# orjfickel/Small-Project-UV-Robot-Ray-Tracer

Measured on AMD Instinct MI355X. Metric: Mray/s (extend+shade) on C046_1.glb 1920x1080x8-bounce, higher is better.
Workload: dtype f32; 1 GPU; testroomopt.glb (stand-in for the absent rooms/C046_1.glb), 2073600 photons/launch x 8 waves, lamp 0 of lange_route.xml, SEED_0=0; step = reset + generate + extend of all waves (batched), accumulate + shade replayed per wave + sync; triangles=44866, mode=batched, launch_pipelining=True, flavour=0, seed_mode=0, wide_bvh=False, parallelism=1 GPU, self_comm=False, high_priority_stream=False, full=False

## Files before the change

small-project-uv-robot-ray-tracer_amd/csrc/uvrt_kernels.hip:

```cpp
#include "uvrt_device.h"

namespace uvrt {


__device__ __forceinline__ uint32_t coherence_key(uint32_t qphi, uint32_t qy, uint32_t qo,
                                                  int bphi, int by, int bo)
{
    uint32_t key = 0;
    while (bphi > 0 || by > 0 || bo > 0) {
        if (bphi > 0) { --bphi; key = (key << 1) | ((qphi >> bphi) & 1u); }
        if (by > 0) { --by; key = (key << 1) | ((qy >> by) & 1u); }
        if (bo > 0) { --bo; key = (key << 1) | ((qo >> bo) & 1u); }
    }
    return key;
}

__global__ __launch_bounds__(256) void k_generate(GenParams p)
{
    helper_priority(p.prio);
    if (blockIdx.x >= p.ray_blocks) {
        const int j = (int)(blockIdx.x - p.ray_blocks) * 256 + threadIdx.x;
        if (j < p.prep_npairs) prepare_record6(p.prep_pairs, p.prep_recs, p.lx, p.lz, p.prep_npairs, j, p.prep_perm);
        return;
    }
    const int64_t i = (int64_t)blockIdx.x * 256 + threadIdx.x;
    if (i >= p.n) return;
    const int64_t gid = p.first_gid + i;
    float r0;
    double x, y;
    const float4 ray = generate_ray(p.lx, p.ly, p.lz, p.light_length, gid, p.seed_prev, p.seed_next, p.seed_mode, r0, x, y);
    const float diry = ray.y;
    p.rays[i] = ray;

    if (p.keyrank) {
        const float fx = (float)x, fy = (float)y;
        const float ax = fabsf(fx), ay = fabsf(fy);
        float t = ay / (ax + ay + 1e-30f);
        float ang = fx >= 0.0f ? (fy >= 0.0f ? t : 4.0f - t) : (fy >= 0.0f ? 2.0f - t : 2.0f + t);
        const uint32_t nphi = 1u << p.bits_phi, ny = 1u << p.bits_y, no = 1u << p.bits_o;
        uint32_t qphi = min((uint32_t)(ang * (0.25f * (float)nphi)), nphi - 1);
        uint32_t qy = min((uint32_t)((diry + 1.0f) * (0.5f * (float)ny)), ny - 1);
        uint32_t qo = min((uint32_t)(r0 * (float)no), no - 1);
        const uint32_t key = coherence_key(qphi, qy, qo, p.bits_phi, p.bits_y, p.bits_o);
        const uint32_t rank = atomicAdd(&p.hist[key], 1u);
        p.keyrank[i] = make_uint2(key, rank);
    }
}

__global__ __launch_bounds__(256) void k_generate_batch(GenBatchParams p)
{
    helper_priority(p.prio);
    const int64_t i = (int64_t)blockIdx.x * 256 + threadIdx.x;
    if (i >= p.n) return;
    const int k = blockIdx.y;
    float r0;
    double x, y;
    p.rays[(int64_t)k * p.n_pad + i] = generate_ray(p.lx[k], p.ly[k], p.lz[k], p.light_length, p.first_gid + i,
                                                    p.seed_prev[k], p.seed_next[k], p.seed_mode, r0, x, y);
}

__global__ __launch_bounds__(64) void k_dedupe_mark(GenDedupeParams p)
{
    helper_priority(p.prio);
    constexpr int32_t W = DEDUPE_MARK_KEYS;
    __shared__ uint32_t s_table[W];
    const int lane = threadIdx.x, K = p.g.count;
    const uint32_t nb = (uint32_t)((p.gn + DD_SLOTS - 1) / DD_SLOTS);
    const int32_t lo = (int32_t)(p.g.first_gid > 1 ? p.g.first_gid : 1), hi = (int32_t)(p.g.first_gid + p.g.n);
    const int32_t c0 = (int32_t)p.g0, c1 = (int32_t)(p.g0 + p.gn);
    if ((int32_t)blockIdx.x >= p.gap_strip0[p.gaps]) {
        static_assert(DEDUPE_PERIODIC_WORDS % 64 == 0 && DEDUPE_PERIODIC_WORDS <= W, "the words fit the key table's LDS in whole rounds");
#pragma unroll
        for (int i = 0; i < DEDUPE_PERIODIC_WORDS; i += 64) s_table[i + lane] = p.per.words[i + lane];
        __syncthreads();
        const uint32_t t = (blockIdx.x - (uint32_t)p.gap_strip0[p.gaps]) * 64u + (uint32_t)lane;
        if (t < (uint32_t)K * nb) {
            const uint32_t k = t / nb, b = t - k * nb;
            const int32_t x0 = c0 + (int32_t)(b * (uint32_t)DD_SLOTS), x1 = min(x0 + DD_SLOTS, c1);
            const uint32_t owners = dedupe_periodic_owners(p.g, p.per, s_table, (int)k, max(x0, 1), x1);
            if (owners != 0u) atomicAdd(&p.block_counts[t], owners);
        }
        return;
    }
    int gap = 0;
    while (gap + 1 < p.gaps && (int32_t)blockIdx.x >= p.gap_strip0[gap + 1]) ++gap;
    const int64_t gap_lo = p.gap_key[gap];
    const uint32_t gap_keys = p.gap_keys[gap];
    const int64_t gap_tiles = (int64_t)((gap_keys + (uint32_t)W - 1u) / (uint32_t)W);
    const int64_t tile0 = (int64_t)((int32_t)blockIdx.x - p.gap_strip0[gap]) * p.strip_tiles;
    const int64_t tile1 = tile0 + p.strip_tiles < gap_tiles ? tile0 + p.strip_tiles : gap_tiles;
    int32_t run_lo = hi, run_hi = hi, key0 = 0;
    uint32_t seed1 = 0u;
    if (lane < K) {
        run_lo = dedupe_strip_first(p.g, lane, gap_lo + tile0 * W);
        seed1 = dedupe_seed1(p.g, lane);
        key0 = p.g.key0[lane];
    }
    uint32_t cnt_block = 0u, cnt = 0u;
    const auto add_owners = [&](int j, uint32_t block, uint32_t owners) { atomicAdd(&p.block_counts[(size_t)j * nb + block], owners); };
    const auto count_owners = [&](int j, uint32_t block, uint32_t owners) {
        if (lane == j && owners != 0u) {
            if (block != cnt_block) {
                if (cnt != 0u) add_owners(j, cnt_block, cnt);
                cnt_block = block;
                cnt = 0u;
            }
            cnt += owners;
        }
    };
    for (int64_t tile = tile0; tile < tile1; ++tile) {
        const int64_t t0 = gap_lo + tile * W;
        const int32_t w = (int32_t)min((uint32_t)W, gap_keys - (uint32_t)(tile * W));
        static_assert(W % 64 == 0, "the wave zeroes the table in whole rounds");
#pragma unroll
        for (int i = 0; i < W; i += 64) s_table[i + lane] = 0u;
        __syncthreads();
        for (int j = 0; j < K; ++j) {
            int32_t base = __builtin_amdgcn_readlane(run_lo, j);
            const uint32_t seed = (uint32_t)__builtin_amdgcn_readlane((int)seed1, j);
            for (;;) {
                const int32_t g = base + lane;
                bool in = false;
                if (g < hi) {
                    const int32_t key = dedupe_key1_of(p.g, seed, g);
                    in = dedupe_in_tile(key, t0, w);
                    if (in) dedupe_tile_insert_run(s_table, dedupe_tile_slot(key, t0), j, dedupe_run_twice(p.g, seed, g, key, lo, hi));
                }
                const int32_t n_in = (int32_t)__popcll(__builtin_amdgcn_ballot_w64(in));
                base += n_in;
                if (n_in < 64) break;
            }
            if (lane == j) run_hi = base;
        }
        const bool holds0 = lane < K && dedupe_tile_holds_key0(p.g, key0, t0, w);
        if (holds0) dedupe_tile_insert(s_table, dedupe_tile_slot(key0, t0), lane);
        __syncthreads();
        for (int j = 0; j < K; ++j) {
            const int32_t a = max(__builtin_amdgcn_readlane(run_lo, j), c0), b = min(__builtin_amdgcn_readlane(run_hi, j), c1);
            const uint32_t seed = (uint32_t)__builtin_amdgcn_readlane((int)seed1, j);
            for (int32_t base = a; base < b; base += 64) {
                const int32_t g = base + lane;
                const uint32_t fb = (uint32_t)(base - c0) / (uint32_t)DD_SLOTS;
                uint32_t mask = 0u, blk = fb;
                if (g < b) {
                    const uint32_t slot = dedupe_tile_slot(dedupe_key1_of(p.g, seed, g), t0);
                    mask = dedupe_tile_resolve(slot < (uint32_t)w ? s_table[slot] : DEDUPE_MANY, j);
                    p.tmp[(int64_t)j * p.gn + (g - c0)] = mask;
                    blk = (uint32_t)(g - c0) / (uint32_t)DD_SLOTS;
                }
                const int32_t last = min(base + 63, b - 1);
                if ((uint32_t)(last - c0) / (uint32_t)DD_SLOTS == fb) {
                    count_owners(j, fb, (uint32_t)__popcll(__builtin_amdgcn_ballot_w64(mask != 0u)));
                } else {
                    const uint32_t n0 = (uint32_t)__popcll(__builtin_amdgcn_ballot_w64(mask != 0u && blk == fb));
                    const uint32_t n1 = (uint32_t)__popcll(__builtin_amdgcn_ballot_w64(mask != 0u && blk != fb));
                    count_owners(j, fb, n0);
                    count_owners(j, fb + 1u, n1);
                }
            }
        }
        if (c0 == 0 && holds0) {
            const uint32_t mask = dedupe_tile_resolve(s_table[dedupe_tile_slot(key0, t0)], lane);
            p.tmp[(int64_t)lane * p.gn] = mask;
            if (mask != 0u) add_owners(lane, 0u, 1u);
        }
        run_lo = run_hi;
        __syncthreads();
    }
    if (lane < K && cnt != 0u) add_owners(lane, cnt_block, cnt);
}

__global__ __launch_bounds__(256) void k_dedupe_scan(uint32_t* block_counts, uint32_t* total, uint32_t* deposits, uint32_t nblocks, int prio)
{
    helper_priority(prio);
    __shared__ uint32_t s_part[256];
    const uint32_t tid = threadIdx.x;
    if (tid == 0u) *deposits = 0u;
    const uint32_t per = (nblocks + 255u) / 256u;
    const uint32_t lo = min(tid * per, nblocks), hi = min(lo + per, nblocks);
    uint32_t sum = 0;
    for (uint32_t b = lo; b < hi; ++b) sum += block_counts[b];
    s_part[tid] = sum;
    __syncthreads();
    for (uint32_t off = 1; off < 256u; off <<= 1) {
        const uint32_t v = tid >= off ? s_part[tid - off] : 0u;
        __syncthreads();
        s_part[tid] += v;
        __syncthreads();
    }
    uint32_t run = s_part[tid] - sum;
    for (uint32_t b = lo; b < hi; ++b) {
        const uint32_t c = block_counts[b];
        block_counts[b] = run;
        run += c;
    }
    if (tid == 255u) *total = s_part[255];
}

__global__ __launch_bounds__(256) void k_dedupe_write(GenDedupeParams p)
{
    helper_priority(p.prio);
    __shared__ uint32_t s_cnt[DD_ROUNDS][4];
    __shared__ uint32_t s_slot_mask[DEDUPE_CLASS_SLOTS], s_slot_word[DEDUPE_CLASS_SLOTS], s_dep;
    if (threadIdx.x < (unsigned)DEDUPE_CLASS_SLOTS) {
        s_slot_mask[threadIdx.x] = p.cls.slot_mask[threadIdx.x];
        s_slot_word[threadIdx.x] = p.cls.slot_word[threadIdx.x];
    }
    if (threadIdx.x == 0) s_dep = 0u;
    const bool classes = p.cls.count > 0;
    uint32_t dep = 0u;
    const int k = blockIdx.y;
    const uint32_t wv = threadIdx.x >> 6;
    static_assert(256 % DEDUPE_PERIOD_MAX == 0, "a thread's rounds share their residue");
    uint32_t near = 0u, worded = 0u;
    bool inside = false;
    const uint32_t seed1 = dedupe_seed1(p.g, k);
    const int32_t gid0 = (int32_t)(p.g0 + (int64_t)blockIdx.x * DD_SLOTS) + (int32_t)threadIdx.x;
    if (p.per.count > 0) {
        const int32_t x0 = max((int32_t)(p.g0 + (int64_t)blockIdx.x * DD_SLOTS), 1);
        const int32_t x1 = (int32_t)min(p.g0 + ((int64_t)blockIdx.x + 1) * DD_SLOTS, p.g0 + p.gn);
        const int32_t ka = __builtin_amdgcn_readfirstlane(dedupe_key1_of(p.g, seed1, x0));
        const int32_t kb = __builtin_amdgcn_readfirstlane(dedupe_key1_of(p.g, seed1, x1 - 1));
#pragma unroll
        for (int s = 0; s < DEDUPE_PERIODIC_STRATA; ++s) {
            const int32_t A = p.per.key_lo[s], B = A + (int32_t)p.per.keys[s];
            if (s < p.per.count && kb >= A && ka < B) {
                near |= 1u << s;
                inside = ka >= A && kb < B;
            }
        }
    }
    uint32_t mask[DD_ROUNDS], rank[DD_ROUNDS];
#pragma unroll
    for (int r = 0; r < DD_ROUNDS; ++r) mask[r] = 0u;
    for (uint32_t left = near; left != 0u; left &= left - 1u) {
        const int s = __builtin_ctz(left);
        const int32_t A = p.per.key_lo[s], P = p.per.period[s];
        const uint32_t len = p.per.keys[s];
        const uint32_t* w = &p.per.words[p.per.word_off[s] + k * P];
        const int32_t res = gid0 & (P - 1);
        uint32_t word = 0u;
#pragma unroll
        for (int q = 0; q < DEDUPE_PERIOD_MAX; ++q) {
            const uint32_t wq = w[q];
            if (res == q) word = wq;
        }
#pragma unroll
        for (int r = 0; r < DD_ROUNDS; ++r) {
            const int64_t i = (int64_t)blockIdx.x * DD_SLOTS + r * 256 + threadIdx.x;
            const int32_t g = gid0 + r * 256;
            if (i < p.gn && g >= 1 && (inside || (uint32_t)dedupe_key1_of(p.g, seed1, g) - (uint32_t)A < len)) {
                mask[r] = word;
                worded |= 1u << r;
            }
        }
    }
    uint32_t pos = p.block_counts[(size_t)k * gridDim.x + blockIdx.x];
#pragma unroll
    for (int r = 0; r < DD_ROUNDS; ++r) {
        const int64_t i = (int64_t)blockIdx.x * DD_SLOTS + r * 256 + threadIdx.x;
        if (!((worded >> r) & 1u) && i < p.gn) mask[r] = p.tmp[(int64_t)k * p.gn + i];
        const unsigned long long owners = __builtin_amdgcn_ballot_w64(mask[r] != 0u);
        rank[r] = __builtin_amdgcn_mbcnt_hi((uint32_t)(owners >> 32), __builtin_amdgcn_mbcnt_lo((uint32_t)owners, 0u));
        if ((threadIdx.x & 63u) == 0u) s_cnt[r][wv] = (uint32_t)__popcll(owners);
    }
    __syncthreads();
    if (threadIdx.x == 0) p.block_counts[(size_t)k * gridDim.x + blockIdx.x] = 0u;
#pragma unroll
    for (int r = 0; r < DD_ROUNDS; ++r) {
        for (uint32_t w = 0; w < 4u; ++w) {
            if (w == wv && mask[r] != 0u) {
                const int64_t i = (int64_t)blockIdx.x * DD_SLOTS + r * 256 + threadIdx.x;
                float r0;
                double x, y;
                p.rays[pos + rank[r]] = generate_ray(p.g.lx, p.g.ly, p.g.lz, p.light_length, p.g0 + i, p.g.seed_prev[k],
                                                     p.g.seed_next[k], p.g.seed_mode, r0, x, y);
                const uint32_t word = ((worded >> r) & 1u) ? mask[r] : dedupe_deposit_word(classes, s_slot_mask, s_slot_word, mask[r]);
                p.masks[pos + rank[r]] = word;
                dep += (uint32_t)dedupe_word_deposits(classes, word);
            }
            pos += s_cnt[r][w];
        }
    }
    if (dep != 0u) atomicAdd(&s_dep, dep);
    __syncthreads();
    if (threadIdx.x == 0 && s_dep != 0u) atomicAdd(p.deposits, s_dep);
}

__global__ __launch_bounds__(1024) void k_scan_bins(uint32_t* hist, uint32_t* bin_start,
                                                    int32_t nbins)
{
    __shared__ uint32_t s_part[1024];
    const int tid = threadIdx.x;
    const int per = (nbins + 1023) / 1024;
    const int lo = tid * per, hi = min(lo + per, nbins);
    uint32_t sum = 0;
    for (int b = lo; b < hi; ++b) sum += hist[b];
    s_part[tid] = sum;
    __syncthreads();
    for (int off = 1; off < 1024; off <<= 1) {
        uint32_t v = tid >= off ? s_part[tid - off] : 0u;
        __syncthreads();
        s_part[tid] += v;
        __syncthreads();
    }
    uint32_t run = s_part[tid] - sum;
    for (int b = lo; b < hi; ++b) {
        const uint32_t c = hist[b];
        bin_start[b] = run;
        hist[b] = 0;
        run += c;
    }
}

__global__ __launch_bounds__(256) void k_scatter(const float4* __restrict__ rays,
                                                 const uint2* __restrict__ keyrank,
                                                 const uint32_t* __restrict__ bin_start,
                                                 float4* __restrict__ sorted,
                                                 uint32_t* __restrict__ order, int64_t n)
{
    const int64_t i = (int64_t)blockIdx.x * 256 + threadIdx.x;
    if (i >= n) return;
    const uint2 kr = keyrank[i];
    const uint32_t pos = bin_start[kr.x] + kr.y;
    const float4 r = rays[i];
    sorted[pos] = r;
    order[pos] = (uint32_t)i;
}


__global__ __launch_bounds__(256) void k_accumulate(double* __restrict__ photon_map,
                                                    double* __restrict__ max_map,
                                                    int32_t* __restrict__ counts, int32_t replicas,
                                                    int64_t stride, float time_step, int32_t T, int prio)
{
    helper_priority(prio);
    const int g = blockIdx.x * 256 + threadIdx.x;
    const int i = g >> 2, part = g & 3;
    int32_t total = 0;
    if (i < T) {
        for (int r = part; r < replicas; r += 4) {
            total += counts[r * stride + i];
            counts[r * stride + i] = 0;
        }
    }
    total += __builtin_amdgcn_mov_dpp(total, 0xb1, 0xf, 0xf, true);
    total += __builtin_amdgcn_mov_dpp(total, 0x4e, 0xf, 0xf, true);
    if (i >= T || part != 0) return;
    const double c = (double)total;
    photon_map[i] = photon_map[i] + c * (double)time_step;
    const double m = max_map[i];
    max_map[i] = m < c ? c : m;
}

__global__ __launch_bounds__(256) void k_fold_counts(int32_t* __restrict__ counts, int32_t replicas,
                                                     int64_t stride, int32_t T)
{
    const int i = blockIdx.x * 256 + threadIdx.x;
    if (i >= T) return;
    int32_t total = counts[i];
    for (int r = 1; r < replicas; ++r) {
        total += counts[r * stride + i];
        counts[r * stride + i] = 0;
    }
    counts[i] = total;
}

__device__ __forceinline__ void heatmap(float intensity, float& r, float& g, float& b)
{
    const float minDosageColor = 0.5f;
    const float upperHalfColor = 0.75f;
    const float lowerHalfColor = 0.25f;
    if (intensity > minDosageColor) {
        if (intensity > upperHalfColor) {
            r = 1.0f; g = (1.0f - intensity) / (1.0f - upperHalfColor); b = 0.0f;
        } else {
            r = (intensity - minDosageColor) / (upperHalfColor - minDosageColor);
            g = 1.0f; b = 0.0f;
        }
    } else {
        if (intensity > lowerHalfColor) {
            r = 0.0f; g = 1.0f;
            b = (minDosageColor - intensity) / (minDosageColor - lowerHalfColor);
        } else {
            r = 0.0f; g = intensity / lowerHalfColor; b = 1.0f;
        }
    }
}

__global__ __launch_bounds__(256) void k_fold_planes(int32_t* __restrict__ planes, int32_t* __restrict__ folded,
                                                     int32_t replicas, int32_t T, int prio)
{
    helper_priority(prio);
    const int g = blockIdx.x * 256 + threadIdx.x;
    const int i = g >> 2, part = g & 3;
    int32_t* pl = planes + (int64_t)blockIdx.y * replicas * T;
    int32_t total = 0;
    if (i < T) {
        for (int r = part; r < replicas; r += 4) {
            total += pl[(int64_t)r * T + i];
            pl[(int64_t)r * T + i] = 0;
        }
    }
    total += __builtin_amdgcn_mov_dpp(total, 0xb1, 0xf, 0xf, true);
    total += __builtin_amdgcn_mov_dpp(total, 0x4e, 0xf, 0xf, true);
    if (i < T && part == 0) folded[(int64_t)blockIdx.y * T + i] = total;
}

__device__ __forceinline__ int32_t take_class_plane(int32_t* pl, int32_t replicas, int64_t replica_stride, int i, int part, bool in)
{
    int32_t total = 0;
    if (in) {
        for (int r = part; r < replicas; r += 4) {
            total += pl[(int64_t)r * replica_stride + i];
            pl[(int64_t)r * replica_stride + i] = 0;
        }
    }
    total += __builtin_amdgcn_mov_dpp(total, 0xb1, 0xf, 0xf, true);
    total += __builtin_amdgcn_mov_dpp(total, 0x4e, 0xf, 0xf, true);
    return total;
}

__global__ __launch_bounds__(256) void k_fold_classes(FoldClassParams p)
{
    helper_priority(p.prio);
    const int g = blockIdx.x * 256 + threadIdx.x;
    const int i = g >> 2, part = g & 3;
    const bool in = i < p.T;
    for (int c = 0; c < p.ncls; ++c) {
        const int32_t total = take_class_plane(p.planes + (int64_t)(p.nplanes + c) * p.plane_stride, p.cls_replicas, p.T, i, part, in);
        if (!in || part != 0 || total == 0) continue;
        for (uint64_t m = p.launches[c]; m != 0ull; m &= m - 1ull) p.folded[(int64_t)__builtin_ctzll(m) * p.T + i] += total;
    }
}

__global__ __launch_bounds__(256) void k_replay_batch(ReplayParams p)
{
    helper_priority(p.prio);
    const int g = blockIdx.x * 256 + threadIdx.x;
    const int i = g >> 2, part = g & 3;
    const bool in = i < p.bound;
    double pm = 0, mm = 0;
    if (in && part == 0) { pm = p.photon_map[i]; mm = p.max_map[i]; }
    extern __shared__ int32_t s_cls[];
    const int ncls = p.is_folded ? 0 : p.ncls;
    for (int c = 0; c < ncls; ++c) {
        const int32_t total = take_class_plane(p.planes + (int64_t)(p.nplanes + c) * p.plane_stride, p.cls_replicas, p.T, i, part, in);
        if (part == 0) s_cls[c * 64 + (threadIdx.x >> 2)] = total;
    }
    for (int k = 0; k < p.count; ++k) {
        const ReplayOp op = p.ops[k];
        int32_t total = 0;
        if (p.is_folded) {
            if (in && part == 0) {
                int32_t* f = p.folded + (int64_t)op.plane * p.T + i;
                total = *f;
                *f = 0;
            }
        } else {
            if (in) {
                int32_t* pl = p.planes + (int64_t)op.plane * p.plane_stride;
                for (int r = part; r < p.replicas; r += 4) {
                    total += pl[(int64_t)r * p.T + i];
                    pl[(int64_t)r * p.T + i] = 0;
                }
            }
            total += __builtin_amdgcn_mov_dpp(total, 0xb1, 0xf, 0xf, true);
            total += __builtin_amdgcn_mov_dpp(total, 0x4e, 0xf, 0xf, true);
        }
        if (!in || part != 0) continue;
        if (ncls > 0)
            for (uint64_t m = p.class_of[k]; m != 0ull; m &= m - 1ull) total += s_cls[__builtin_ctzll(m) * 64 + (threadIdx.x >> 2)];
        const double c = (double)total;
        pm = pm + c * (double)op.duration;
        mm = mm < c ? c : mm;
        if (op.shade) {
            const double num = (double)op.scaled_power * (op.which_map ? mm : pm);
            const float den = p.area[i] * (float)op.photons_per_light;
            const float dose = (float)(num / (double)den);
            p.dosage[i] = dose;
            const float maxValue = op.min_value * 2;
            const float norm = dose / maxValue;
            float r, gg, b;
            if (op.threshold_view && norm < 0.5f) { r = 0.0f; gg = 0.0f; b = norm * 2.0f; }
            else heatmap(norm, r, gg, b);
            float* col = p.color + (int64_t)i * 9;
            col[0] = r; col[1] = gg; col[2] = b;
            col[3] = r; col[4] = gg; col[5] = b;
            col[6] = r; col[7] = gg; col[8] = b;
        }
    }
    if (in && part == 0) { p.photon_map[i] = pm; p.max_map[i] = mm; }
}

__global__ __launch_bounds__(256) void k_add_counts(int32_t* __restrict__ dst, const int32_t* __restrict__ src, int64_t n)
{
    const int64_t i = (int64_t)blockIdx.x * 256 + threadIdx.x;
    if (i < n) dst[i] += src[i];
}

__global__ __launch_bounds__(256) void k_reset(double* __restrict__ photon_map,
                                               double* __restrict__ max_map,
                                               int32_t* __restrict__ counts, int32_t replicas,
                                               int64_t stride, float* __restrict__ color,
                                               int32_t reset_color, int32_t T, int prio)
{
    helper_priority(prio);
    const int i = blockIdx.x * 256 + threadIdx.x;
    if (i >= T) return;
    photon_map[i] = 0;
    max_map[i] = 0;
    for (int r = 0; r < replicas; ++r) counts[r * stride + i] = 0;
    if (!reset_color) return;
    for (int k = 0; k < 9; ++k) color[(int64_t)i * 9 + k] = 0.0f;
}

__global__ __launch_bounds__(256) void k_prepare_scene(const float4* __restrict__ tris64,
                                                       const uint32_t* __restrict__ tri_idx,
                                                       LeafTri* __restrict__ ltris,
                                                       float* __restrict__ area, int32_t T)
{
    const int i = blockIdx.x * 256 + threadIdx.x;
    if (i >= T) return;
    {
        const uint32_t id = tri_idx[i];
        const float4 v0 = tris64[(int64_t)id * 4 + 0], v1 = tris64[(int64_t)id * 4 + 1],
                     v2 = tris64[(int64_t)id * 4 + 2];
        LeafTri t;
        t.v0_id = make_float4(v0.x, v0.y, v0.z, __uint_as_float(id));
        t.e1 = make_float4(v1.x - v0.x, v1.y - v0.y, v1.z - v0.z, 0.0f);
        t.e2 = make_float4(v2.x - v0.x, v2.y - v0.y, v2.z - v0.z, 0.0f);
        ltris[i] = t;
    }
    {
        const float4 v0 = tris64[(int64_t)i * 4 + 0], v1 = tris64[(int64_t)i * 4 + 1],
                     v2 = tris64[(int64_t)i * 4 + 2];
        const float ax = v0.x - v1.x, ay = v0.y - v1.y, az = v0.z - v1.z;
        const float bx = v0.x - v2.x, by = v0.y - v2.y, bz = v0.z - v2.z;
        const float cx = ay * bz - az * by;
        const float cy = az * bx - ax * bz;
        const float cz = ax * by - ay * bx;
        area[i] = sqrtf(cx * cx + cy * cy + cz * cz) / 2.0f;
    }
}

__global__ __launch_bounds__(256) void k_compute_dosage(const double* __restrict__ map,
                                                        float* __restrict__ dosage,
                                                        const float* __restrict__ area,
                                                        int32_t photons_per_light,
                                                        float scaled_power, int32_t T)
{
    const int i = blockIdx.x * 256 + threadIdx.x;
    if (i >= T) return;
    const double num = (double)scaled_power * map[i];
    const float den = area[i] * (float)photons_per_light;
    dosage[i] = (float)(num / (double)den);
}

__global__ __launch_bounds__(256) void k_dosage_to_color(const float* __restrict__ dosage,
                                                         float* __restrict__ color,
                                                         float min_value, int32_t threshold_view,
                                                         int32_t T)
{
    const int i = blockIdx.x * 256 + threadIdx.x;
    if (i >= T) return;
    const float maxValue = min_value * 2;
    const float norm = dosage[i] / maxValue;
    float r, g, b;
    if (threshold_view && norm < 0.5f) { r = 0.0f; g = 0.0f; b = norm * 2.0f; }
    else heatmap(norm, r, g, b);
    float* c = color + (int64_t)i * 9;
    c[0] = r; c[1] = g; c[2] = b;
    c[3] = r; c[4] = g; c[5] = b;
    c[6] = r; c[7] = g; c[8] = b;
}

__device__ __forceinline__ void shade_one(int i, double map_value, float* __restrict__ dosage, const float* __restrict__ area,
                                          float* __restrict__ color, int32_t photons_per_light, float scaled_power,
                                          float min_value, int32_t threshold_view)
{
    const double num = (double)scaled_power * map_value;
    const float den = area[i] * (float)photons_per_light;
    const float dose = (float)(num / (double)den);
    dosage[i] = dose;
    const float maxValue = min_value * 2;
    const float norm = dose / maxValue;
    float r, g, b;
    if (threshold_view && norm < 0.5f) { r = 0.0f; g = 0.0f; b = norm * 2.0f; }
    else heatmap(norm, r, g, b);
    float* c = color + (int64_t)i * 9;
    c[0] = r; c[1] = g; c[2] = b;
    c[3] = r; c[4] = g; c[5] = b;
    c[6] = r; c[7] = g; c[8] = b;
}

__global__ __launch_bounds__(256) void k_shade(const double* __restrict__ map, float* __restrict__ dosage,
                                               const float* __restrict__ area, float* __restrict__ color,
                                               int32_t photons_per_light, float scaled_power,
                                               float min_value, int32_t threshold_view, int32_t T, int prio)
{
    helper_priority(prio);
    const int i = blockIdx.x * 256 + threadIdx.x;
    if (i >= T) return;
    shade_one(i, map[i], dosage, area, color, photons_per_light, scaled_power, min_value, threshold_view);
}

__global__ __launch_bounds__(256) void k_accumulate_shade(double* __restrict__ photon_map, double* __restrict__ max_map,
                                                          int32_t* __restrict__ counts, int32_t replicas, int64_t stride,
                                                          float time_step, float* __restrict__ dosage,
                                                          const float* __restrict__ area, float* __restrict__ color,
                                                          int32_t which_map, int32_t photons_per_light, float scaled_power,
                                                          float min_value, int32_t threshold_view, int32_t T, int prio)
{
    helper_priority(prio);
    const int g = blockIdx.x * 256 + threadIdx.x;
    const int i = g >> 2, part = g & 3;
    int32_t total = 0;
    if (i < T) {
        for (int r = part; r < replicas; r += 4) {
            total += counts[r * stride + i];
            counts[r * stride + i] = 0;
        }
    }
    total += __builtin_amdgcn_mov_dpp(total, 0xb1, 0xf, 0xf, true);
    total += __builtin_amdgcn_mov_dpp(total, 0x4e, 0xf, 0xf, true);
    if (i >= T || part != 0) return;
    const double c = (double)total;
    const double sum = photon_map[i] + c * (double)time_step;
    photon_map[i] = sum;
    const double m = max_map[i];
    const double mx = m < c ? c : m;
    max_map[i] = mx;
    shade_one(i, which_map ? mx : sum, dosage, area, color, photons_per_light, scaled_power, min_value, threshold_view);
}

__global__ __launch_bounds__(64) void k_clock_probe(unsigned long long* out, unsigned long long ticks)
{
    const unsigned long long r0 = __builtin_amdgcn_s_memrealtime();
    const unsigned long long t0 = __builtin_amdgcn_s_memtime();
    unsigned long long r1 = r0;
    while (r1 - r0 < ticks) {
        __builtin_amdgcn_s_sleep(32);
        r1 = __builtin_amdgcn_s_memrealtime();
    }
    const unsigned long long t1 = __builtin_amdgcn_s_memtime();
    r1 = __builtin_amdgcn_s_memrealtime();
    if (threadIdx.x == 0) { out[0] = t1 - t0; out[1] = r1 - r0; }
}

void launch_clock_probe(unsigned long long* out, unsigned long long ticks, hipStream_t s)
{
    hipLaunchKernelGGL(k_clock_probe, dim3(1), dim3(64), 0, s, out, ticks);
}

__global__ __launch_bounds__(256) void k_export_rays(const float4* __restrict__ rays,
                                                     const uint2* __restrict__ hits,
                                                     float4* __restrict__ out, float ox,
                                                     float oz, int64_t first, int64_t count)
{
    const int64_t i = (int64_t)blockIdx.x * 256 + threadIdx.x;
    if (i >= count) return;
    const float4 rec = rays[first + i];
    uint2 h = make_uint2(__float_as_uint(1e30f), 0u);
    if (hits) h = hits[first + i];
    out[i * 2 + 0] = make_float4(rec.x, rec.y, rec.z, ox);
    out[i * 2 + 1] = make_float4(rec.w, oz, __uint_as_float(h.x), __uint_as_float(h.y));
}


static inline unsigned blocks_for(int64_t n, int per) { return (unsigned)((n + per - 1) / per); }

void launch_generate(const GenParams& p0, hipStream_t s)
{
    GenParams p = p0;
    p.ray_blocks = p.n > 0 ? blocks_for(p.n, 256) : 0u;
    const unsigned prep_blocks = p.prep_recs ? blocks_for(p.prep_npairs, 256) : 0u;
    if (p.ray_blocks + prep_blocks == 0) return;
    hipLaunchKernelGGL(k_generate, dim3(p.ray_blocks + prep_blocks), dim3(256), 0, s, p);
}

void launch_generate_batch(const GenBatchParams& p, hipStream_t s)
{
    if (p.n <= 0 || p.count <= 0) return;
    hipLaunchKernelGGL(k_generate_batch, dim3(blocks_for(p.n, 256), (unsigned)p.count), dim3(256), 0, s, p);
}

void launch_dedupe_mark(const GenDedupeParams& p, hipStream_t s)
{
    if (p.gn <= 0 || p.g.count <= 0 || (p.gaps <= 0 && p.per.count <= 0) || p.strip_tiles <= 0) return;
    const unsigned count_groups = p.per.count > 0 ? blocks_for((int64_t)p.g.count * blocks_for(p.gn, DD_SLOTS), 64) : 0u;
    hipLaunchKernelGGL(k_dedupe_mark, dim3((unsigned)p.gap_strip0[p.gaps] + count_groups), dim3(64), 0, s, p);
}

void launch_generate_dedupe(const GenDedupeParams& p, hipStream_t s)
{
    if (p.gn <= 0 || p.g.count <= 0) return;
    const dim3 grid(blocks_for(p.gn, DD_SLOTS), (unsigned)p.g.count);
    launch_dedupe_mark(p, s);
    hipLaunchKernelGGL(k_dedupe_scan, dim3(1), dim3(256), 0, s, p.block_counts, p.total, p.deposits, grid.x * grid.y, (int)p.prio);
    hipLaunchKernelGGL(k_dedupe_write, grid, dim3(256), 0, s, p);
}

void launch_fold_planes(int32_t* planes, int32_t* folded, int32_t nplanes, int32_t replicas, int32_t T, int prio, hipStream_t s)
{
    if (nplanes <= 0 || T <= 0) return;
    hipLaunchKernelGGL(k_fold_planes, dim3(blocks_for((int64_t)T * 4, 256), (unsigned)nplanes), dim3(256), 0, s, planes,
                       folded, replicas, T, prio);
}

void launch_replay_batch(const ReplayParams& p, hipStream_t s)
{
    if (p.count <= 0 || p.bound <= 0) return;
    const size_t lds = p.is_folded ? 0 : (size_t)p.ncls * 64 * sizeof(int32_t);
    hipLaunchKernelGGL(k_replay_batch, dim3(blocks_for((int64_t)p.bound * 4, 256)), dim3(256), lds, s, p);
}

void launch_fold_classes(const FoldClassParams& p, hipStream_t s)
{
    if (p.ncls <= 0 || p.T <= 0) return;
    hipLaunchKernelGGL(k_fold_classes, dim3(blocks_for((int64_t)p.T * 4, 256)), dim3(256), 0, s, p);
}

void launch_add_counts(int32_t* dst, const int32_t* src, int64_t n, hipStream_t s)
{
    if (n <= 0) return;
    hipLaunchKernelGGL(k_add_counts, dim3(blocks_for(n, 256)), dim3(256), 0, s, dst, src, n);
}

void launch_scan_bins(uint32_t* hist, uint32_t* bin_start, int32_t nbins, hipStream_t s)
{
    hipLaunchKernelGGL(k_scan_bins, dim3(1), dim3(1024), 0, s, hist, bin_start, nbins);
}

void launch_scatter(const float4* rays, const uint2* keyrank, const uint32_t* bin_start,
                    float4* sorted, uint32_t* order, int64_t n, hipStream_t s)
{
    if (n <= 0) return;
    hipLaunchKernelGGL(k_scatter, dim3(blocks_for(n, 256)), dim3(256), 0, s, rays, keyrank,
                       bin_start, sorted, order, n);
}

void launch_accumulate(double* photon_map, double* max_map, int32_t* counts, int32_t replicas,
                       int64_t stride, float time_step, int32_t T, int prio, hipStream_t s)
{
    if (T <= 0) return;
    hipLaunchKernelGGL(k_accumulate, dim3(blocks_for((int64_t)T * 4, 256)), dim3(256), 0, s, photon_map,
                       max_map, counts, replicas, stride, time_step, T, prio);
}

void launch_fold_counts(int32_t* counts, int32_t replicas, int64_t stride, int32_t T, hipStream_t s)
{
    if (T <= 0 || replicas <= 1) return;
    hipLaunchKernelGGL(k_fold_counts, dim3(blocks_for(T, 256)), dim3(256), 0, s, counts, replicas,
                       stride, T);
}

void launch_reset(double* photon_map, double* max_map, int32_t* counts, int32_t replicas,
                  int64_t stride, float* color, int32_t reset_color, int32_t T, int prio, hipStream_t s)
{
    if (T <= 0) return;
    hipLaunchKernelGGL(k_reset, dim3(blocks_for(T, 256)), dim3(256), 0, s, photon_map, max_map,
                       counts, replicas, stride, color, reset_color, T, prio);
}

void launch_compute_dosage(const double* map, float* dosage, const float* area,
                           int32_t photons_per_light, float scaled_power, int32_t T,
                           hipStream_t s)
{
    if (T <= 0) return;
    hipLaunchKernelGGL(k_compute_dosage, dim3(blocks_for(T, 256)), dim3(256), 0, s, map, dosage,
                       area, photons_per_light, scaled_power, T);
}

void launch_shade(const double* map, float* dosage, const float* area, float* color, int32_t photons_per_light,
                  float scaled_power, float min_value, int32_t threshold_view, int32_t T, int prio, hipStream_t s)
{
    if (T <= 0) return;
    hipLaunchKernelGGL(k_shade, dim3(blocks_for(T, 256)), dim3(256), 0, s, map, dosage, area, color,
                       photons_per_light, scaled_power, min_value, threshold_view, T, prio);
}

void launch_accumulate_shade(double* photon_map, double* max_map, int32_t* counts, int32_t replicas, int64_t stride,
                             float time_step, float* dosage, const float* area, float* color, int32_t which_map,
                             int32_t photons_per_light, float scaled_power, float min_value, int32_t threshold_view,
                             int32_t T, int prio, hipStream_t s)
{
    if (T <= 0) return;
    hipLaunchKernelGGL(k_accumulate_shade, dim3(blocks_for((int64_t)T * 4, 256)), dim3(256), 0, s, photon_map, max_map, counts,
                       replicas, stride, time_step, dosage, area, color, which_map, photons_per_light, scaled_power, min_value,
                       threshold_view, T, prio);
}

void launch_dosage_to_color(const float* dosage, float* color, float min_value,
                            int32_t threshold_view, int32_t T, hipStream_t s)
{
    if (T <= 0) return;
    hipLaunchKernelGGL(k_dosage_to_color, dim3(blocks_for(T, 256)), dim3(256), 0, s, dosage,
                       color, min_value, threshold_view, T);
}

void launch_prepare_scene(const float4* tris64, const uint32_t* tri_idx, LeafTri* ltris,
                          float* area, int32_t T, hipStream_t s)
{
    if (T <= 0) return;
    hipLaunchKernelGGL(k_prepare_scene, dim3(blocks_for(T, 256)), dim3(256), 0, s, tris64,
                       tri_idx, ltris, area, T);
}

void launch_export_rays(const float4* rays, const uint2* hits, void* out32, float ox, float oz,
                        int64_t first, int64_t count, hipStream_t s)
{
    if (count <= 0) return;
    hipLaunchKernelGGL(k_export_rays, dim3(blocks_for(count, 256)), dim3(256), 0, s, rays, hits,
                       (float4*)out32, ox, oz, first, count);
}

}
```

Baseline: 17540 Mray/s.

## Compact survivor ray generation in dedupe write and vectorize dedupe block scan

```diff
diff --git a/small-project-uv-robot-ray-tracer_amd/csrc/uvrt_kernels.hip b/small-project-uv-robot-ray-tracer_amd/csrc/uvrt_kernels.hip
--- a/small-project-uv-robot-ray-tracer_amd/csrc/uvrt_kernels.hip
+++ b/small-project-uv-robot-ray-tracer_amd/csrc/uvrt_kernels.hip
@@ -177,6 +177,61 @@
     const uint32_t tid = threadIdx.x;
     if (tid == 0u) *deposits = 0u;
     const uint32_t per = (nblocks + 255u) / 256u;
+    if (per <= 16u) {
+        const uint32_t quads = (per + 3u) / 4u;
+        const uint32_t first = tid * quads * 4u;
+        uint32_t c[16];
+#pragma unroll
+        for (uint32_t q = 0; q < 4u; ++q) {
+            const uint32_t b = first + q * 4u;
+            uint4 v = make_uint4(0u, 0u, 0u, 0u);
+            if (q < quads) {
+                if (b + 4u <= nblocks) {
+                    v = *reinterpret_cast<const uint4*>(block_counts + b);
+                } else {
+                    if (b + 0u < nblocks) v.x = block_counts[b + 0u];
+                    if (b + 1u < nblocks) v.y = block_counts[b + 1u];
+                    if (b + 2u < nblocks) v.z = block_counts[b + 2u];
+                }
+            }
+            c[q * 4u + 0u] = v.x, c[q * 4u + 1u] = v.y, c[q * 4u + 2u] = v.z, c[q * 4u + 3u] = v.w;
+        }
+        uint32_t sum = 0u;
+#pragma unroll
+        for (int i = 0; i < 16; ++i) sum += c[i];
+        uint32_t inc = sum;
+        inc += (uint32_t)__builtin_amdgcn_update_dpp(0, (int)inc, 0x111, 0xf, 0xf, false);
+        inc += (uint32_t)__builtin_amdgcn_update_dpp(0, (int)inc, 0x112, 0xf, 0xf, false);
+        inc += (uint32_t)__builtin_amdgcn_update_dpp(0, (int)inc, 0x114, 0xf, 0xf, false);
+        inc += (uint32_t)__builtin_amdgcn_update_dpp(0, (int)inc, 0x118, 0xf, 0xf, false);
+        inc += (uint32_t)__builtin_amdgcn_update_dpp(0, (int)inc, 0x142, 0xa, 0xf, false);
+        inc += (uint32_t)__builtin_amdgcn_update_dpp(0, (int)inc, 0x143, 0xc, 0xf, false);
+        if ((tid & 63u) == 63u) s_part[tid >> 6] = inc;
+        __syncthreads();
+        const uint32_t w0 = s_part[0], w1 = s_part[1], w2 = s_part[2], w3 = s_part[3];
+        const uint32_t wv = tid >> 6;
+        uint32_t run = inc - sum + (wv > 0u ? w0 : 0u) + (wv > 1u ? w1 : 0u) + (wv > 2u ? w2 : 0u);
+#pragma unroll
+        for (uint32_t q = 0; q < 4u; ++q) {
+            const uint32_t b = first + q * 4u;
+            uint4 v;
+            v.x = run, run += c[q * 4u + 0u];
+            v.y = run, run += c[q * 4u + 1u];
+            v.z = run, run += c[q * 4u + 2u];
+            v.w = run, run += c[q * 4u + 3u];
+            if (q < quads) {
+                if (b + 4u <= nblocks) {
+                    *reinterpret_cast<uint4*>(block_counts + b) = v;
+                } else {
+                    if (b + 0u < nblocks) block_counts[b + 0u] = v.x;
+                    if (b + 1u < nblocks) block_counts[b + 1u] = v.y;
+                    if (b + 2u < nblocks) block_counts[b + 2u] = v.z;
+                }
+            }
+        }
+        if (tid == 255u) *total = w0 + w1 + w2 + w3;
+        return;
+    }
     const uint32_t lo = min(tid * per, nblocks), hi = min(lo + per, nblocks);
     uint32_t sum = 0;
     for (uint32_t b = lo; b < hi; ++b) sum += block_counts[b];
@@ -201,6 +256,7 @@
 {
     helper_priority(p.prio);
     __shared__ uint32_t s_cnt[DD_ROUNDS][4];
+    __shared__ uint16_t s_list[DD_SLOTS];
     __shared__ uint32_t s_slot_mask[DEDUPE_CLASS_SLOTS], s_slot_word[DEDUPE_CLASS_SLOTS], s_dep;
     if (threadIdx.x < (unsigned)DEDUPE_CLASS_SLOTS) {
         s_slot_mask[threadIdx.x] = p.cls.slot_mask[threadIdx.x];
@@ -266,18 +322,16 @@
     }
     __syncthreads();
     if (threadIdx.x == 0) p.block_counts[(size_t)k * gridDim.x + blockIdx.x] = 0u;
+    const uint32_t pos0 = pos;
 #pragma unroll
     for (int r = 0; r < DD_ROUNDS; ++r) {
         for (uint32_t w = 0; w < 4u; ++w) {
             if (w == wv && mask[r] != 0u) {
-                const int64_t i = (int64_t)blockIdx.x * DD_SLOTS + r * 256 + threadIdx.x;
-                float r0;
-                double x, y;
-                p.rays[pos + rank[r]] = generate_ray(p.g.lx, p.g.ly, p.g.lz, p.light_length, p.g0 + i, p.g.seed_prev[k],
-                                                     p.g.seed_next[k], p.g.seed_mode, r0, x, y);
+                const uint32_t slot = pos + rank[r];
                 const uint32_t word = ((worded >> r) & 1u) ? mask[r] : dedupe_deposit_word(classes, s_slot_mask, s_slot_word, mask[r]);
-                p.masks[pos + rank[r]] = word;
+                p.masks[slot] = word;
                 dep += (uint32_t)dedupe_word_deposits(classes, word);
+                s_list[slot - pos0] = (uint16_t)(r * 256 + (int)threadIdx.x);
             }
             pos += s_cnt[r][w];
         }
@@ -285,6 +339,14 @@
     if (dep != 0u) atomicAdd(&s_dep, dep);
     __syncthreads();
     if (threadIdx.x == 0 && s_dep != 0u) atomicAdd(p.deposits, s_dep);
+    const uint32_t n_wg = (uint32_t)__builtin_amdgcn_readfirstlane((int)(pos - pos0));
+    const int64_t gid_wg = p.g0 + (int64_t)blockIdx.x * DD_SLOTS;
+    for (uint32_t e = threadIdx.x; e < n_wg; e += 256u) {
+        float r0;
+        double x, y;
+        p.rays[pos0 + e] = generate_ray(p.g.lx, p.g.ly, p.g.lz, p.light_length, gid_wg + s_list[e], p.g.seed_prev[k],
+                                        p.g.seed_next[k], p.g.seed_mode, r0, x, y);
+    }
 }
 
 __global__ __launch_bounds__(1024) void k_scan_bins(uint32_t* hist, uint32_t* bin_start,
```

After: 17490 Mray/s, median of 2. No clear change (-0.3%).
